# Simple-Robotics/LoIK

Measured on AMD Instinct MI355X. Metric: IK solves/sec to 1e-6 residual, Talos humanoid, batch=65536 per GPU, higher is better.
Workload: dtype f64

## Files before the change

loik_amd/csrc/loik_flat.hpp:

```cpp
#pragma once

#include "loik_lean.hpp"

namespace loikb {

constexpr int FLAT_RED = 8;
constexpr int FLAT_PART = 8;
constexpr int FLAT_JMP = 5;
constexpr int FLAT_MAXA = 16;
constexpr int FOLDW = 10;
constexpr int FLAT_COUNTERS_SLOT_HITS = 12;
constexpr int FLAT_NA_SMALL = 10;
constexpr int FSLOT_ROWS = 8;

struct FlatLane {
  int depth;
  int size;
  int jmp[FLAT_JMP];
  int anc[FLAT_MAXA];
  int red[FLAT_RED];
  int helper;
  int part[FLAT_PART];
};

enum : int { FC_LANE = 0, FC_B = 1, FC_Y = 7, FC_ATY = 13, FC_ATYW = 19, FC_ATBW = 25, FC_DY = 31, FC_DLT = 37, FC_ATYF = 43, FC_AW = 49, FC_A = 85,
              FC_VC = FC_DLT , FCD = 121 };
enum : int { FI_BNORM = 0, FI_TGIN, FI_STY, FI_TOLP, FI_TOLD, FI_DYQP, FI_ATDY, FI_UBP, FI_LBM, FI_C1, FI_C2, FI_PRIMAL, FI_DUAL, FI_DX,
             FI_DZ, FI_MULAST, FI_RED , FISC = FI_RED + 16 };

template <int NA>
__host__ __device__ constexpr int flat_xregion()
{
  int n = XROWS * 9;
  if (NA * WAVE + 2 > n) n = NA * WAVE + 2;
  if (WAVE * FOLDW > n) n = WAVE * FOLDW;
  return (n + 1) & ~1;
}
template <int NA> __host__ __device__ constexpr int flat_off_wl() { return flat_xregion<NA>(); }
template <int NA> __host__ __device__ constexpr int flat_off_nbuf() { return flat_off_wl<NA>() + 2 * (NA + 1) * WAVE; }
template <int NA> __host__ __device__ constexpr int flat_off_pbuf() { return flat_off_nbuf<NA>() + WAVE + 2; }
template <int NA> __host__ __device__ constexpr int flat_off_rbuf() { return flat_off_pbuf<NA>() + WAVE + 2; }
template <int NA> __host__ __device__ constexpr int flat_off_tail() { return flat_off_rbuf<NA>() + WAVE; }

template <typename T, int NA>
__host__ __device__ __forceinline__ size_t flat_lds_bytes(int nc, int G, bool a_shared, bool has_hv)
{
  (void)a_shared;
  const size_t per_inst = (size_t)nc * FCD + FISC;
  const size_t n = (size_t)flat_off_tail<NA>() + (has_hv ? (size_t)WAVE * 6 : 0) + (size_t)(WAVE / G) * per_inst;
  return (n * sizeof(T) + 15) & ~(size_t)15;
}

__device__ __forceinline__ size_t fslotA_at(int idx, int ndec, int dsl, int fblk, int G, int k, int jlane)
{
  (void)G;
  return ((size_t)idx * ndec + dsl) * fblk + (size_t)jlane * 8 + k;
}
__device__ __forceinline__ size_t fslotW_at(int idx, int ndec, int dsl, int fblk, int col)
{
  return ((size_t)idx * ndec + dsl) * fblk + col;
}

template <typename T>
__device__ __forceinline__ void se3_compose_left(const T* Ra, const T* ta, T* R, T* t)
{
  T Rn[9], tn[3];
#pragma unroll
  for (int i = 0; i < 3; ++i) {
#pragma unroll
    for (int j = 0; j < 3; ++j) Rn[3 * i + j] = Ra[3 * i] * R[j] + Ra[3 * i + 1] * R[3 + j] + Ra[3 * i + 2] * R[6 + j];
    tn[i] = ta[i] + Ra[3 * i] * t[0] + Ra[3 * i + 1] * t[1] + Ra[3 * i + 2] * t[2];
  }
#pragma unroll
  for (int k = 0; k < 9; ++k) R[k] = Rn[k];
#pragma unroll
  for (int k = 0; k < 3; ++k) t[k] = tn[k];
}

template <typename T>
__device__ __forceinline__ void flat_world_placement(T* xb, int lane, int jlane, const unsigned int* jrow4, int njmp, T* R, T* t)
{
#pragma unroll 1
  for (int r = 0; r < njmp; ++r) {
    {
      const int jr = (int)(((r < 4 ? jrow4[0] : jrow4[1]) >> (8 * (r & 3))) & 0xFFu);
      T Ra[9], ta[3];
      tail_sync();
      if (jlane < 9) xb[WAVE * 9 + jlane] = (jlane == 0 || jlane == 4 || jlane == 8) ? T(1) : T(0);
#pragma unroll
      for (int k = 0; k < 9; ++k) xb[lane * 9 + k] = R[k];
      tail_sync();
#pragma unroll
      for (int k = 0; k < 9; ++k) Ra[k] = xb[jr * 9 + k];
      tail_sync();
      if (jlane < 3) xb[WAVE * 9 + jlane] = T(0);
#pragma unroll
      for (int k = 0; k < 3; ++k) xb[lane * 9 + k] = t[k];
      tail_sync();
#pragma unroll
      for (int k = 0; k < 3; ++k) ta[k] = xb[jr * 9 + k];
      se3_compose_left(Ra, ta, R, t);
    }
  }
  tail_sync();
}

template <typename T>
__device__ __forceinline__ void flat_subtree_sum(T* rows, int lane, int jlane, int lim, int size, int nscan, const T* x, T* S)
{
  tail_sync();
  if (jlane < 6) rows[WAVE * 6 + jlane] = T(0);
  T B[6];
#pragma unroll
  for (int k = 0; k < 6; ++k) { B[k] = x[k]; S[k] = T(0); }
  int pos = lane;
  for (int k = 0; k < nscan; ++k) {
    tail_sync();
#pragma unroll
    for (int c = 0; c < 6; ++c) rows[lane * 6 + c] = B[c];
    tail_sync();
    const bool take = (size >> k) & 1;
    const int ra = take ? pos : WAVE;
    const int nx = lane + (1 << k);
    const int rb = nx < lim ? nx : WAVE;
    T a[6], b[6];
#pragma unroll
    for (int c = 0; c < 6; ++c) a[c] = rows[ra * 6 + c];
#pragma unroll
    for (int c = 0; c < 6; ++c) b[c] = rows[rb * 6 + c];
#pragma unroll
    for (int c = 0; c < 6; ++c) { S[c] += a[c]; B[c] += b[c]; }
    pos += take ? (1 << k) : 0;
  }
}

template <typename T>
__device__ __forceinline__ void flat_path_sum(T* rows, int lane, int jlane, const unsigned int* jrow4, int njmp, T* y)
{
  tail_sync();
  if (jlane < 6) rows[WAVE * 6 + jlane] = T(0);
#pragma unroll 1
  for (int r = 0; r < njmp; ++r) {
    {
      const int jr = (int)(((r < 4 ? jrow4[0] : jrow4[1]) >> (8 * (r & 3))) & 0xFFu);
      tail_sync();
#pragma unroll
      for (int c = 0; c < 6; ++c) rows[lane * 6 + c] = y[c];
      tail_sync();
      T a[6];
#pragma unroll
      for (int c = 0; c < 6; ++c) a[c] = rows[jr * 6 + c];
#pragma unroll
      for (int c = 0; c < 6; ++c) y[c] += a[c];
    }
  }
}

template <typename T>
__device__ __forceinline__ void actinv_force(const T* R, const T* t, const T* F, T* o)
{
  T c[3], d[3];
  cross3(t, F, c);
#pragma unroll
  for (int k = 0; k < 3; ++k) d[k] = F[3 + k] - c[k];
  mat3t_vec(R, F, o);
  mat3t_vec(R, d, o + 3);
}

template <typename T, int NMAX>
__device__ __forceinline__ void flat_fold8(T* rows, int lane, int gbase, int jlane, int lgG, const T* in, T* out)
{
  tail_sync();
  T* row = rows + lane * FOLDW;
#pragma unroll
  for (int q = 0; q < 8; ++q) row[q] = in[q];
  tail_sync();
  const int q = jlane & 7;
  const bool ismax = q < NMAX;
  const int nparts = 1 << (lgG - 3);
  {
    const T* col = rows + (gbase + (jlane >> 3)) * FOLDW + q;
    T a[8];
#pragma unroll
    for (int u = 0; u < 8; ++u) a[u] = col[u * nparts * FOLDW];
    const T m = tmax(tmax(tmax(a[0], a[1]), tmax(a[2], a[3])), tmax(tmax(a[4], a[5]), tmax(a[6], a[7])));
    T sm = a[0];
#pragma unroll
    for (int u = 1; u < 8; ++u) sm += a[u];
    row[8] = (NMAX >= 8 || ismax) ? m : sm;
  }
  tail_sync();
  {
    const T* col = rows + (gbase + q) * FOLDW + 8;
    T a[8];
#pragma unroll
    for (int p = 0; p < 8; ++p) a[p] = (p < 4 || lgG > 5) ? col[p * 8 * FOLDW] : T(0);
    const T m = tmax(tmax(tmax(a[0], a[1]), tmax(a[2], a[3])), tmax(tmax(a[4], a[5]), tmax(a[6], a[7])));
    T sm = a[0];
#pragma unroll
    for (int p = 1; p < 8; ++p) sm += a[p];
    row[9] = (NMAX >= 8 || ismax) ? m : sm;
  }
  tail_sync();
#pragma unroll
  for (int u = 0; u < 8; ++u) out[u] = rows[(gbase + u) * FOLDW + 9];
}

__device__ __forceinline__ unsigned int opaque(unsigned int x) { asm volatile("" : "+v"(x)); return x; }
// ... 538 lines not shown
      for (; kk + 2 < nscan; ++kk) {
        put_rows();
        tail_sync();
        scan_step(kk);
      }
      if (kk >= nscan) {
        tail_sync();
        part_v();
      } else {
        put_rows();
        tail_sync();
        const int wv = 1 << kk;
        const bool take0 = (size >> kk) & 1, take1 = (size >> (kk + 1)) & 1;
        const int p1 = pos + (take0 ? wv : 0);
        const int r0 = take0 ? pos : WAVE, r1 = take1 ? p1 : WAVE, r2 = take1 ? p1 + wv : WAVE;
        T a[6], b[6], c2[6];
#pragma unroll
        for (int c = 0; c < 6; ++c) a[c] = xb[r0 * 6 + c];
#pragma unroll
        for (int c = 0; c < 6; ++c) b[c] = xb[r1 * 6 + c];
#pragma unroll
        for (int c = 0; c < 6; ++c) c2[c] = xb[r2 * 6 + c];
        part_v();
#pragma unroll
        for (int c = 0; c < 6; ++c) SEn[c] += a[c] + (b[c] + c2[c]);
      }
      tail_sync();
      TAIL_TP(4)
#pragma unroll
      for (int k = 0; k < 6; ++k) Fw[k] = (P.rho + href_s) * SEn[k] - P.rho * SE[k];
      if (has_hv) {
#pragma unroll
        for (int k = 0; k < 6; ++k) Fw[k] -= shv[lane * 6 + k];
      }
      for (int c = 0; c < L.nc; ++c) {
        const T* c_ = cdi + c * cs;
        const T m = cmask(c);
#pragma unroll
        for (int k = 0; k < 6; ++k) Fw[k] += m * c_[FC_ATYF + k];
      }
      actinv_force(R0, t0, Fw, fi);
      si = dot6_halves(Sw, Fw);
#pragma unroll
      for (int k = 0; k < 6; ++k) SE[k] = SEn[k];
    }
    TAIL_TP(5)
    {
      T df[6];
#pragma unroll
      for (int k = 0; k < 6; ++k) df[k] = fi[k] - f[k];
      l_dfis = mass * inf6(df);
      si += w;
      l_stf = tabs(si);
      l_dstf = tabs(si - s);
      s = si;
#pragma unroll
      for (int k = 0; k < 6; ++k) f[k] = fi[k];
    }
    TAIL_TP(3)
    T red[8];
    {
      T in[8] = {tmax(l_prt, l_prs), tmax(l_dualv, l_stf), tmax(l_dvis, l_dnu), l_dz,
                 tmax(l_dfis, tmax(l_dyis, l_dw)), tmax(l_dg, l_dstf), l_up, l_lm};
      flat_fold8<T, 6>(xb, lane, gbase, jlane, lgG, in, red);
    }
    T ntol_p = T(0), ntol_d = T(0);
    if (P.tol_rel != T(0)) {
      T in2[8] = {tmax(l_av, l_nu), tmax(tmax(l_hrefv, l_g), l_stf), T(0), T(0), T(0), T(0), T(0), T(0)}, r2[8];
      flat_fold8<T, 8>(xb, lane, gbase, jlane, lgG, in2, r2);
      ntol_p = r2[0]; ntol_d = r2[1];
    }
    TAIL_TP(6)
    const T primal = red[0], dual = red[1], dx = red[2], dz = red[3], dyqp = red[4], atdy = red[5], ubp = red[6], lbm = red[7];
    const T mu_used = mu;
    const bool fixed = P.mode & MODE_FIXED_ITERS;
    const bool in_tail = (status & ST_TAIL) != 0;
    const bool logic = act && !fixed && !in_tail;
    const T tol_p = P.tol_abs + P.tol_rel * tmax(ntol_p, isc[FI_BNORM]);
    const T tol_d = P.tol_abs + P.tol_rel * tmax(ntol_d, P.Hv_inf_norm);
    const int itn = iter + (act ? 1 : 0);
    const bool conv = logic && (primal < tol_p) && (dual < tol_d);
    const bool feas_chk = logic && itn > 1;
    const bool c1 = atdy <= P.tol_primal_inf * dyqp, c2 = (ubp + lbm) <= P.tol_primal_inf * dyqp;
    const bool infeas = feas_chk && c1 && c2;
    const bool enter_tail = infeas && !conv;
    const bool upd = logic && !conv && !infeas;
    const bool mu_up = upd && (primal > T(10) * dual), mu_dn = upd && !mu_up && (dual > T(10) * primal);
    const bool tail_stop = !(dx >= P.tol_tail_solve || dz >= P.tol_tail_solve) || itn >= P.max_iter;
    const bool stop = act && (conv || ((enter_tail || in_tail) && tail_stop) || ((upd || fixed) && itn + 1 >= P.max_iter));
    iter = itn;
    status |= (conv ? ST_CONVERGED : 0) | (infeas ? ST_PRIMAL_INF : 0) | (enter_tail ? ST_TAIL : 0) | (stop ? ST_DONE : 0);
    tail_it = enter_tail ? 0 : (act && in_tail ? tail_it + 1 : tail_it);
    mu = mu_up ? mu * T(10) : (mu_dn ? mu * T(0.1) : mu);
    kexp += (mu_up ? 1 : 0) - (mu_dn ? 1 : 0);
    nflip += (mu_up || mu_dn) ? 1 : 0;
    done = done || stop;
    const bool finishing = stop;
    const bool leaving = done && has_inst;
    if (LOG) {
      T inl[8] = {l_prt, l_prs, l_stf, l_dualv, T(0), T(0), T(0), T(0)}, rl[8];
      flat_fold8<T, 8>(xb, lane, gbase, jlane, lgG, inl, rl);
      const int row = itn - 1;
      if (act && !in_tail && jlane == 0 && row < Bf.log_cap) {
        const double vals[9] = {(double)rl[0], (double)rl[1], (double)primal, (double)rl[2], (double)rl[3], (double)dual,
                                (double)mu_used, (double)(P.mu_scale * mu_used), (double)mu_used};
#pragma unroll
        for (int l = 0; l < 9; ++l) Bf.log[((size_t)l * Bf.log_B + lidx) * Bf.log_cap + row] = vals[l];
      }
    }
    if (__any(finishing || enter_tail)) {
      if ((finishing || enter_tail) && jlane == 0) {
        isc[FI_PRIMAL] = primal; isc[FI_DUAL] = dual; isc[FI_DX] = dx; isc[FI_DZ] = dz; isc[FI_MULAST] = mu_used;
        if (logic) { isc[FI_TOLP] = tol_p; isc[FI_TOLD] = tol_d; }
        if (feas_chk) {
          isc[FI_C1] = (T)(c1 ? 1 : 0); isc[FI_C2] = (T)(c2 ? 1 : 0); isc[FI_DYQP] = dyqp; isc[FI_ATDY] = atdy; isc[FI_UBP] = ubp; isc[FI_LBM] = lbm;
        }
      }
    }
    if (__any(finishing)) {
      T in1[8] = {l_prt, l_prs, l_stf, l_dvis, l_dnu, l_dfis, l_dyis, l_dw}, in2[8] = {l_av, l_nu, l_hrefv, l_g, l_dualv, T(0), T(0), T(0)};
      T r1[8], r2[8];
      flat_fold8<T, 8>(xb, lane, gbase, jlane, lgG, in1, r1);
      flat_fold8<T, 8>(xb, lane, gbase, jlane, lgG, in2, r2);
      if (finishing && jlane == 0) {
#pragma unroll
        for (int k = 0; k < 8; ++k) isc[FI_RED + k] = r1[k];
#pragma unroll
        for (int k = 0; k < 5; ++k) isc[FI_RED + 8 + k] = r2[k];
      }
      tail_sync();
    }
    if (leaving) {
      store_instance();
      need_load = true;
    }
    TAIL_TP(7)
  }
#ifdef LOIKB_TAIL_PROF
  if (blockIdx.x == 0 && threadIdx.x == 0) {
    for (int k = 0; k < 8; ++k) g_tail_prof[k] = prof_[k];
    for (int k = 8; k < 12; ++k) g_tail_prof[2 + k] = prof_[k];
    g_tail_prof[8] = n_wave_iters;
    g_tail_prof[9] = (clock64() - clk0_) * 100000ull / (wall_clock64() - wall0_ + 1);
  }
#endif
  if (lane == 0) atomicAdd(&Bf.counters[5], n_wave_iters);
  if (jlane == 0) {
    atomicAdd(&Bf.counters[6], n_slot_loads >> 16);
    atomicAdd(&Bf.counters[FLAT_COUNTERS_SLOT_HITS], n_slot_hits);
    atomicOr(&Bf.counters[LEAN_DECADES_SEEN], n_slot_loads & 0xFFFFu);
  }
}

template <typename T, int NA>
__global__ void __launch_bounds__(WAVE)
k_fslots(const Params<T> P, const Bufs<T> Bf, const JointDesc* __restrict__ jd, const TailTopo* __restrict__ topo,
         const int* __restrict__ child_list, const FlatLane* __restrict__ fl, int maxdepth, int nanc, int frows, int njmp,
         const int* __restrict__ slots, int nslots, int G, T* __restrict__ fslots, int kexp_lo, int ndec, int dw0, int nw,
         unsigned int* __restrict__ fmask)
{
  extern __shared__ __attribute__((aligned(16))) unsigned char smem_raw[];
  const Layout& L = P.L;
  constexpr int HX = 22;
  T* xch = reinterpret_cast<T*>(smem_raw);
  T* swt = xch + (WAVE + 1) * HX;
  T* ata_l = swt + (WAVE + 1) * 6;
  T* mutab = ata_l + (size_t)(WAVE / G) * P.L.nc * 21;
  T* lb = xch;
  const int lane = threadIdx.x;
  const int ipw = WAVE / G;
  const int sub = lane / G, jlane = lane % G, gbase = sub * G;
  const int nblk = gridDim.x, xcd = blockIdx.x & 7, rnd = blockIdx.x >> 3;
  const int blk = xcd * (nblk >> 3) + (xcd < (nblk & 7) ? xcd : (nblk & 7)) + rnd;
  const int idx = blk * ipw + sub;
  const bool has_inst = idx < nslots;
  const bool isj_lane = jlane < L.nb;
  const bool isj = has_inst && isj_lane;
  const int jl = isj_lane ? jlane : 0;
  const int sidx = slots[has_inst ? idx : 0];
  char* ip = lane_ptr<T>(Bf.tiles, L, sidx);
  int depth, fcol, arow[NA];
  T Sw[6];
  bool has_parent;
  int cslot;
  T base0[21];
  {
    const JointDesc d = jd[jl + 1];
    const FlatLane F = fl[jlane];
    depth = isj_lane ? F.depth : 0;
    fcol = F.helper >> 8;
    has_parent = !(d.flags & JF_PARENT_ROOT);
    cslot = isj_lane ? d.cslot : -1;
    unsigned int jrow4[(FLAT_JMP + 3) / 4] = {0u, 0u};
#pragma unroll
    for (int r = 0; r < FLAT_JMP; ++r) jrow4[r >> 2] |= (unsigned int)(F.jmp[r] >= 0 ? gbase + F.jmp[r] : WAVE) << (8 * (r & 3));
#pragma unroll
    for (int k = 0; k < NA; ++k) arow[k] = (k < FLAT_MAXA && F.anc[k] >= 0) ? gbase + F.anc[k] : WAVE;
    const char* rec = ip + (size_t)jl * JREC * pair_bytes<T>();
    const typename Vec2<T>::type cs = ldp<T>(rec, JP_CS);
    T R0[9], t0[3];
    joint_xform<T>(d, rec, cs.x, cs.y, R0, t0);
    if (!isj_lane) {
#pragma unroll
      for (int k = 0; k < 9; ++k) R0[k] = (k % 4 == 0) ? T(1) : T(0);
#pragma unroll
      for (int k = 0; k < 3; ++k) t0[k] = T(0);
    }
    flat_world_placement<T>(xch, lane, jlane, jrow4, njmp, R0, t0);
    const bool rev = d.flags & JF_REVOLUTE;
    const int jflags_h = d.flags;
    const T pitch_h = (d.flags & JF_HELICAL) ? (T)d.pitch : T(0);
    T ax[3], ra3[3], c[3];
#pragma unroll
    for (int k = 0; k < 3; ++k) ax[k] = isj_lane ? (T)d.axis[k] : T(0);
    mat3_vec(R0, ax, ra3);
    cross3(t0, ra3, c);
#pragma unroll
    for (int k = 0; k < 3; ++k) { Sw[k] = rev ? c[k] : ra3[k]; Sw[3 + k] = rev ? ra3[k] : T(0); }
    if (jflags_h & JF_HELICAL) {
#pragma unroll
      for (int k = 0; k < 3; ++k) Sw[k] += pitch_h * ra3[k];
    }
#pragma unroll
    for (int k = 0; k < 6; ++k) swt[lane * 6 + k] = Sw[k];
    if (lane < 6) swt[WAVE * 6 + lane] = T(0);
    {
      const T mass = (!isj_lane || (d.flags & JF_MASSLESS)) ? T(0) : T(1);
      T hb[21];
#pragma unroll
      for (int a = 0; a < 6; ++a)
#pragma unroll
        for (int b2 = a; b2 < 6; ++b2)
          hb[sym(a, b2)] = mass * ((a == b2 ? P.rho : T(0)) + (P.href_tab ? P.href_tab[(size_t)(jl + 1) * HREF_ROW + 6 * a + b2] : P.Href[6 * a + b2]));
      congr_sym(R0, t0, hb, base0);
    }
    if (cslot >= 0) {
      const char* crec = ip + (size_t)(L.off_c + cslot * L.crec) * pair_bytes<T>();
      T at[21], atw[21];
      for (int k = 0; k < 21; ++k)
        at[k] = (P.mode & MODE_A_SHARED) ? Bf.uni[L.nc * 36 + cslot * 21 + k]
                                         : *reinterpret_cast<const T*>(crec + (size_t)(CP_ATA + k / 2) * pair_bytes<T>() + (k & 1) * sizeof(T));
      congr_sym(R0, t0, at, atw);
#pragma unroll
      for (int k = 0; k < 21; ++k) ata_l[(sub * L.nc + cslot) * 21 + k] = atw[k];
    }
  }
  const TailTopo tp = topo[jl + 1];
  constexpr int NCH_REG = 3;
  int chl[NCH_REG];
#pragma unroll
  for (int c = 0; c < NCH_REG; ++c) chl[c] = (isj_lane && c < tp.nchild) ? gbase + child_list[tp.child_start + c] : WAVE;
  if (lane < ndec && lane < 16) mutab[lane] = (T)flat_decade_mu((double)P.mu0, kexp_lo + lane);
  tail_sync();
  if (lane < HX) xch[WAVE * HX + lane] = T(0);
  if (fmask != nullptr && has_inst && jlane == 0) fmask[sidx] = (nw >= 32 ? 0xFFFFu : ((1u << nw) - 1u)) << dw0;
  {
    const int lag = maxdepth - depth;
    tail_sync();
    for (int st = 0; st < maxdepth + nw - 1; ++st) {
      const int dsl = dw0 + st - lag;
      const bool on = isj && depth > 0 && dsl >= dw0 && dsl < dw0 + nw;
      T hh[21];
#pragma unroll
      for (int k = 0; k < 21; ++k) hh[k] = base0[k];
      const bool any2 = __any(on && tp.nchild > 1), any3 = __any(on && tp.nchild > 2);
      if (on) {
#pragma unroll
        for (int c = 0; c < NCH_REG; ++c) {
          if ((c == 1 && !any2) || (c == 2 && !any3)) continue;
          const T* x = xch + chl[c] * HX;
#pragma unroll
          for (int k = 0; k < 21; ++k) hh[k] += x[k];
        }
#pragma unroll 1
        for (int c = NCH_REG; c < tp.nchild; ++c) {
          const T* x = xch + (gbase + child_list[tp.child_start + c]) * HX;
#pragma unroll
          for (int k = 0; k < 21; ++k) hh[k] += x[k];
        }
      }
      tail_sync();
      if (on) {
        const T mu = mutab[dsl];
        const T mu_eq = P.mu_scale * mu, mu_in = mu;
        if (cslot >= 0) {
          const T* at = ata_l + (sub * L.nc + cslot) * 21;
#pragma unroll
          for (int k = 0; k < 21; ++k) hh[k] += mu_eq * at[k];
        }
        T U[6], UD[6];
        symv(hh, Sw, U);
        const T dinv = T(1) / (dot6_halves(Sw, U) + mu_in);
#pragma unroll
        for (int k = 0; k < 6; ++k) UD[k] = U[k] * dinv;
#pragma unroll
        for (int k = 0; k < 6; ++k) fslots[fslotA_at(sidx, ndec, dsl, frows, G, k, jlane)] = UD[k];
        fslots[fslotA_at(sidx, ndec, dsl, frows, G, 6, jlane)] = dinv;
        if (has_parent) {
          T* x = xch + lane * HX;
#pragma unroll
          for (int a = 0; a < 6; ++a)
#pragma unroll
            for (int b2 = a; b2 < 6; ++b2) x[sym(a, b2)] = hh[sym(a, b2)] - UD[a] * U[b2];
        }
      }
      tail_sync();
    }
  }
  lb[NA * WAVE + lane] = T(0);
  __builtin_amdgcn_s_waitcnt(0);
  tail_sync();
  for (int dsl = dw0; dsl < dw0 + nw; ++dsl) {
    T UDw[6], dinv = T(0);
#pragma unroll
    for (int k = 0; k < 6; ++k) UDw[k] = isj ? fslots[fslotA_at(sidx, ndec, dsl, frows, G, k, jlane)] : T(0);
    if (isj) dinv = fslots[fslotA_at(sidx, ndec, dsl, frows, G, 6, jlane)];
    T Lc[NA], Wc[NA];
#pragma unroll
    for (int k = 0; k < NA; ++k) {
      Lc[k] = dot6_halves(swt + arow[k] * 6, UDw);
      Wc[k] = T(0);
    }
    tail_sync();
#pragma unroll
    for (int k = 0; k < NA; ++k) lb[k * WAVE + lane] = Lc[k];
    tail_sync();
#pragma unroll
    for (int k = NA - 1; k >= 0; --k) {
      T acc = Lc[k];
#pragma unroll
      for (int k2 = k + 1; k2 < NA; ++k2) acc += lb[k * WAVE + arow[k2]] * Wc[k2];
      Wc[k] = (k < depth - 1) ? -acc : T(0);
    }
    tail_sync();
    if (isj) {
      const size_t base = fslotW_at(sidx, ndec, dsl, frows, fcol);
#pragma unroll
      for (int k = 0; k < NA; ++k)
        if (k < depth - 1) fslots[base + k] = Wc[k];
      fslots[base + depth - 1] = dinv;
    }
  }
}

template <typename T>
__global__ void k_rebuild_ud(char* tiles, Layout L, const JointDesc* __restrict__ jd, const T* __restrict__ uni, T rho, T mu_scale,
                             const T* __restrict__ href_tab, int a_shared, int B, T* __restrict__ scratch)
{
  const int b = blockIdx.x * blockDim.x + threadIdx.x;
  if (b >= B) return;
  char* lp = lane_ptr<T>(tiles, L, b);
  char* srec = lp + (size_t)L.off_s * pair_bytes<T>();
  if (*elem_ptr<T>(srec, SP_TAG, 0) != T(-2)) return;
  const T mu = *elem_ptr<T>(srec, SP_ST, 1);
  const T mu_eq = mu_scale * mu, mu_in = mu;
  T* o = scratch + (size_t)b * L.nb * 21;
  for (int i = 1; i <= L.nb; ++i) {
    for (int r = 0; r < 6; ++r)
      for (int c = r; c < 6; ++c)
        o[(i - 1) * 21 + sym(r, c)] = (jd[i].flags & JF_MASSLESS) ? T(0) : ((r == c ? rho : T(0)) + href_tab[(size_t)i * HREF_ROW + 6 * r + c]);
    if (jd[i].cslot >= 0) {
      const int cs = jd[i].cslot;
      for (int k = 0; k < 21; ++k) {
        const T a = a_shared ? uni[L.nc * 36 + cs * 21 + k]
                             : *elem_ptr<T>(lp + (size_t)(L.off_c + cs * L.crec) * pair_bytes<T>(), CP_ATA + k / 2, k & 1);
        o[(i - 1) * 21 + k] += mu_eq * a;
      }
    }
  }
  for (int i = L.nb; i >= 1; --i) {
    const JointDesc d = jd[i];
    T hh[21], U[6], UD[6], R[9], t[3], part[21];
    for (int k = 0; k < 21; ++k) hh[k] = o[(i - 1) * 21 + k];
    const int a0 = (d.flags & JF_REVOLUTE) ? 3 : 0;
    const T ax0 = (T)d.axis[0], ax1 = (T)d.axis[1], ax2 = (T)d.axis[2];
    for (int k = 0; k < 6; ++k) U[k] = hh[sym(k, a0)] * ax0 + hh[sym(k, a0 + 1)] * ax1 + hh[sym(k, a0 + 2)] * ax2;
    T sus = ax0 * U[a0] + ax1 * U[a0 + 1] + ax2 * U[a0 + 2];
    if (d.flags & JF_HELICAL) {
      const T ph = (T)d.pitch;
      for (int k = 0; k < 6; ++k) U[k] += ph * (hh[sym(k, 0)] * ax0 + hh[sym(k, 1)] * ax1 + hh[sym(k, 2)] * ax2);
      sus = (ax0 * U[3] + ax1 * U[4] + ax2 * U[5]) + ph * (ax0 * U[0] + ax1 * U[1] + ax2 * U[2]);
    }
    const T dd = T(1) / (sus + mu_in);
    for (int k = 0; k < 6; ++k) UD[k] = U[k] * dd;
    char* rec = lp + (size_t)(i - 1) * JREC * pair_bytes<T>();
    st6<T>(rec, JP_UD, UD);
    st_hi<T>(rec, JP_R, dd);
    {
      T vv[6], ff[6], hv[6];
      ld6<T>(rec, JP_V, vv);
      ld6<T>(rec, JP_F, ff);
      symv(hh, vv, hv);
      for (int k = 0; k < 6; ++k) ff[k] -= hv[k];
      st6<T>(rec, JP_P, ff);
    }
    if (d.parent == 0) continue;
    for (int r = 0; r < 6; ++r)
      for (int c = r; c < 6; ++c) hh[sym(r, c)] -= UD[r] * U[c];
    const typename Vec2<T>::type cs = ldp<T>(rec, JP_CS);
    joint_xform<T>(d, rec, cs.x, cs.y, R, t);
    congr_sym(R, t, hh, part);
    for (int k = 0; k < 21; ++k) o[(d.parent - 1) * 21 + k] += part[k];
  }
  *elem_ptr<T>(srec, SP_TAG, 0) = mu;
  *elem_ptr<T>(srec, SP_ST, 0) = (T)((int)*elem_ptr<T>(srec, SP_ST, 0) | ST_PFULL);
}

}
```

loik_amd/csrc/loik_host.hip:

```cpp
#include "loik_device.hpp"
#include "loik_tail.hpp"
#include "loik_lean.hpp"
#include "loik_flat.hpp"
#include "loik_flat2.hpp"
#include "loik_passes.hpp"
#include "loik_pose.hpp"
#ifdef LOIKB_FLAT_SEPARATE_TU
#include "loik_flat_inst.hpp"
LOIKB_FLAT2_INSTANCES(LOIKB_FLAT2_DECL)
LOIKB_FLAT1_INSTANCES(LOIKB_FLAT1_DECL)
#ifdef LOIKB_TAIL_PROF
int loikb_flat_prof_read(unsigned long long* out, int which, int reset);
#endif
#endif

#include "../../include/loik_amd.h"
#include "../../include/loik_amd_pose.h"

#include <algorithm>
#include <chrono>
#include <cmath>
#include <cstdio>
#include <cstdlib>
#include <cstring>
// ... 1533 lines not shown
  else if (S->f32) pl.why_not_flat = "fp32 solver";
  else if (S->opt.flags & LOIKB_OPT_NO_H_CACHE) pl.why_not_flat = "LOIKB_OPT_NO_H_CACHE (no precomputed factors)";
  else if (flat_any_mu(S) && !flat_any_mu_ok(S))
    pl.why_not_flat = "OSQP penalty rule: mu is off the decade grid, and the in-wave builder is k_flat2's / k_flat1's (17..64 joints, fp64, no logging)";
  else if (S->nb <= 16) pl.why_not_flat = "a small robot (<= 16 joints): k_solve + k_tail are faster on its short solves";
  else if (S->nc > (flat_takes_diagonal(S) ? 10 : S->flat.G / 6)) pl.why_not_flat = "more task constraints than the flat engine's lanes update in one pass";
  else if (pl.flat_waves_cu < (flat_takes_diagonal(S) ? 4 : 6)) pl.why_not_flat = "constraint blocks leave too few wavefronts per CU in LDS";
  else pl.flat = true;
  const bool flat_usable = pl.flat && (!S->href_known || flat_takes_diagonal(S) || href_is_scalar(S));
  pl.tail_max = S->opt.tail_max_instances > 0 ? S->opt.tail_max_instances : ((pl.lean || flat_usable) ? (1 << 20) : 32768);
  const int ntiles = (S->B + WAVE - 1) / WAVE;
  pl.nchunks = (ntiles >= 512 && !pl.lean && !flat_usable) ? 2 : 1;
  if (S->tune.chunks > 0) pl.nchunks = S->tune.chunks;
  pl.nchunks = std::max(1, std::min(pl.nchunks, ntiles));
  {
    auto need_of = [&](const loikb_solver_impl::TeamSched& sc) {
      const int edge = std::max(std::max(sc.nslots, 1) * EDGE_ENT, sc.nw > 1 ? sc.nw * Norms<double>::NALL : 0);
      return (size_t)(edge + std::max(sc.nvslots, 1) * 6) * WAVE * S->esz;
    };
    pl.solve_lds_need = need_of(S->sched[0]);
    pl.solve_ok = pl.solve_lds_need <= (size_t)160 * 1024;
    if (!pl.solve_ok) { pl.tail_max = 1 << 20; pl.nchunks = 1; }
  }
  S->plan = pl;
}

static bool bushy_goes_on_chip(const loikb_solver_impl* S)
{
  return S->nb <= WAVE && S->opt.tail_max_instances >= 0 && S->opt.max_launch_iters <= 0 &&
         !(S->opt.flags & (LOIKB_OPT_NO_COMPACTION | LOIKB_OPT_NO_H_CACHE)) && S->B <= S->plan.tail_max && S->tune.direct_tail;
}

template <typename T>
int run_tail(loikb_solver_impl* S, Chunk* C, Params<T>& P, int cur, int n_cur, int n_live, double* ms_out,
             unsigned long long* iters_out, bool whole_set = false)
{
  loikb_solver_impl::Set& A = C->set[cur];
  const int nw = (n_cur + WAVE - 1) / WAVE;
  int G0 = 8;
  while (G0 < S->nb) G0 <<= 1;
  const bool small_flat = whole_set && cur == 0 && S->chunks.size() == 1 && sizeof(T) == 8 && S->tune.flat_split && flat_applicable(S) && (P.mode & MODE_CACHE_H) &&
                          ((G0 == F2G && S->flat.ok && S->flat.nanc <= FLAT_NA_SMALL) || G0 == WAVE) && n_cur <= S->tune.flat_small_batch &&
                          n_cur >= std::max(1, S->tune.flat_min_batch);
  if (whole_set && small_flat) {
  } else if (whole_set) {
    hipLaunchKernelGGL(k_list_iota, grid1(n_cur), dim3(256), 0, C->stream, C->d_slots, n_cur);
  } else {
    C->h_wave.resize(2 * (size_t)nw + 2);
    int* cnt = C->h_wave.data();
    int* off = cnt + nw + 1;
    HIPCHK(hipMemcpyAsync(cnt, A.wave_live, sizeof(int) * nw, hipMemcpyDeviceToHost, C->stream));
    HIPCHK(hipStreamSynchronize(C->stream));
    int total = 0;
    for (int w = 0; w < nw; ++w) { off[w] = total; total += cnt[w]; }
    if (total != n_live) { g_last_error = "tail: live count mismatch"; return LOIKB_ERR_STATE; }
    HIPCHK(hipMemcpyAsync(A.wave_off, off, sizeof(int) * nw, hipMemcpyHostToDevice, C->stream));
    hipLaunchKernelGGL(k_list_live<T>, dim3(nw), dim3(WAVE), 0, C->stream, A.tiles, S->L, n_cur, A.wave_off, C->d_slots);
  }
  HIPCHK(hipGetLastError());
  Bufs<T> Bf = make_bufs<T>(S, C, cur);
  P.B = n_cur;
  int G = 8;
  while (G < S->nb) G <<= 1;
  const int ipw = WAVE / G;
  int tw = S->tune.tail_waves;
  while (tw > 1 && tw * tail_lds_bytes<T>(S->nc, G) > 160 * 1024) --tw;
  const size_t lds = tw * tail_lds_bytes<T>(S->nc, G);
  if (lds > 160 * 1024) { g_last_error = "tail kernel: constraint data exceeds the LDS of a CU"; return LOIKB_ERR_ARG; }
  if (lds > 64 * 1024) {
    HIPCHK(hipFuncSetAttribute((const void*)k_tail<T, true>, hipFuncAttributeMaxDynamicSharedMemorySize, (int)lds));
    HIPCHK(hipFuncSetAttribute((const void*)k_tail<T, false>, hipFuncAttributeMaxDynamicSharedMemorySize, (int)lds));
  }
  const int cu_share = std::max(1, (int)(S->ncu * (TAIL_WAVES / tw) * ((double)C->B / (double)S->B) + 0.5));
  int n = n_live;
  double total_ms = 0.0;
  unsigned long long iters = 0;
  const bool trace = S->tune.trace;
  const int* list = C->d_slots;
  {
    int ndec = S->plan.ndec, kexp_lo = S->plan.kexp_lo;
    if (S->tune.lean_adapt && S->seen_hi >= S->seen_lo && !(S->opt.flags & LOIKB_OPT_FIXED_ITERS) && !S->opt.logging) {
      const int lo = std::max(kexp_lo, S->seen_lo - 1), hi = std::min(kexp_lo + ndec - 1, S->seen_hi + 1);
      if (hi >= lo) { kexp_lo = lo; ndec = hi - lo + 1; }
    }
    const int ndec_hist = ndec, kexp_lo_hist = kexp_lo;
    const size_t wave_lds = lean_lds_bytes<T>(S->nc, G, S->a_shared);
    const bool flat_one_per_wave = S->tune.flat_split && sizeof(T) == 8 && ((G == F2G && S->flat.ok && S->flat.nanc <= FLAT_NA_SMALL) || G == WAVE);
    const bool flat_ok = flat_applicable(S) && (P.mode & MODE_CACHE_H) && n >= (flat_one_per_wave ? std::max(1, S->tune.flat_min_batch) : 64);
    if (flat_ok) {
      const int nanc = S->flat.nanc;
      const bool small_na = nanc <= FLAT_NA_SMALL;
      const int frows = S->flat.fblk;
      const bool can_build2 = S->tune.flat_build && G == F2G && small_na && sizeof(T) == 8 && S->tune.flat_split && C->d_fmask != nullptr &&
                              !S->opt.logging && !S->per_link && href_is_scalar(S);
      int mur = flat_any_mu(S) ? 1 : (can_build2 ? 2 : 0);
      if (mur == 1) { ndec = 1; kexp_lo = 0; }
      if (mur == 2) { ndec = S->plan.ndec; kexp_lo = S->plan.kexp_lo; }
      const size_t need = (size_t)n_cur * ndec * frows * sizeof(T);
      if (need > C->fslots_bytes) { g_last_error = "internal: decade-slot buffer of the flat engine smaller than the chunk"; return LOIKB_ERR_STATE; }
      const int has_hv = S->Hv_inf_norm != 0.0;
      const size_t flds = small_na ? flat_lds_bytes<T, FLAT_NA_SMALL>(S->nc, G, S->a_shared, has_hv) : flat_lds_bytes<T, FLAT_MAXA>(S->nc, G, S->a_shared, has_hv);
      int lgG = 3;
      while ((1 << lgG) < G) ++lgG;
      const double cu_sh = std::max(1.0, S->ncu * ((double)C->B / (double)S->B));
      const int cap_lat = (int)std::min<size_t>(4, (160 * 1024) / flds) * (int)(cu_sh + 0.5);
      const bool split = S->tune.flat_split && G == F2G && small_na && sizeof(T) == 8;
      const bool one = S->tune.flat_split && G == WAVE && sizeof(T) == 8;
      P.max_launch_iters = S->opt.max_iter + 1;
      const int mode_keep = P.mode;
      if (whole_set && S->zero_state && S->tune.flat_zero_state) P.mode |= MODE_ZERO_STATE;
      const bool queue_ready = small_flat && C->queue_ready && n_cur == S->B;
      C->queue_ready = false;
      if (queue_ready) {}
      else if (small_flat) hipLaunchKernelGGL(k_queue_init_iota, grid1(std::max(C->ring_cap, NCOUNTERS)), dim3(256), 0, C->stream, C->d_ring, C->ring_cap, C->d_slots, n_cur, C->d_counters, NCOUNTERS);
      else HIPCHK(hipMemsetAsync(C->d_counters, 0, NCOUNTERS * sizeof(unsigned int), C->stream));
      const hipEvent_t ev_first = queue_ready ? S->ev_t0 : C->ev_k0;
      if (!queue_ready) HIPCHK(hipEventRecord(C->ev_k0, C->stream));
      const bool ordered = !small_flat && whole_set && list == C->d_slots && n == n_cur && (split || one) && order_usable(S, C, n_cur);
      const bool order_was_stale = ordered && C->order_epoch != S->inputs_epoch;
      if (C->order_holdoff > 0) --C->order_holdoff;
      if (ordered) HIPCHK(hipMemcpyAsync(C->d_slots, C->d_order, sizeof(int) * (size_t)n, hipMemcpyDeviceToDevice, C->stream));
      C->stats.flat_ordered += ordered ? 1 : 0;
      int dw0 = 0, nw = ndec;
      if (mur == 2) {
        int wlo = 0, whi = -1;
        int q = (split && !S->opt.logging) ? flat_slice_for(S, n, ordered) : 0;
        if (q > 0 && (C->d_park == nullptr || (size_t)n_cur * flat2_park_stride(S->nc, true) * sizeof(double) > C->park_bytes)) q = 0;
        const bool win_ok = q > 0 && C->d_park != nullptr;
        if (S->tune.flat_win_n > 0) { wlo = S->tune.flat_win_lo; whi = wlo + S->tune.flat_win_n - 1; }
        else if (S->tune.flat_build == 2 && win_ok && S->end_hist_n > 0) {
          unsigned long long cum = 0;
          int k03 = 99, k97 = 99;
          for (int k = 0; k < 32; ++k) {
            cum += S->end_hist[k];
            if (k03 == 99 && cum * 100 >= 3ull * S->end_hist_n) k03 = k - 16;
            if (k97 == 99 && cum * 100 >= 97ull * S->end_hist_n) k97 = k - 16;
          }
          wlo = std::min(0, k03); whi = std::max(0, k97);
        }
        else if (S->tune.flat_build == 2 && win_ok && n >= 49152) {
          wlo = 0; whi = 4;
        }
        const int lo = std::max(wlo, kexp_lo), hi = std::min(whi, kexp_lo + ndec - 1);
        if (hi >= lo && (hi - lo + 1) < ndec) { dw0 = lo - kexp_lo; nw = hi - lo + 1; }
        else if (S->tune.flat_build == 2) mur = 0;
      }
      if (mur == 0) {
        ndec = ndec_hist; kexp_lo = kexp_lo_hist;
        nw = ndec; dw0 = 0;
      }
      const int win_bits = (int)(((nw >= 16 ? 0xFFFFu : ((1u << nw) - 1u)) << dw0) & 0xFFFFu);
      if (ndec > 0) {
        const dim3 hgrid((unsigned)((n + ipw - 1) / ipw));
        const size_t slds = (std::max((size_t)(WAVE + 1) * 22, (size_t)((small_na ? FLAT_NA_SMALL : FLAT_MAXA) + 1) * WAVE) + (size_t)(WAVE + 1) * 6 +
                             (size_t)ipw * S->nc * 21 + 16) * sizeof(T);
        if (small_na)
          hipLaunchKernelGGL((k_fslots<T, FLAT_NA_SMALL>), hgrid, dim3(WAVE), slds, C->stream, P, Bf, (const JointDesc*)S->d_jd,
                             (const TailTopo*)S->d_topo, (const int*)S->d_child_list, (const FlatLane*)S->flat.d_lanes, S->maxdepth,
                             nanc, frows, S->flat.njmp, list, n, G, (T*)C->d_fslots, kexp_lo, ndec, dw0, nw,
                             mur == 2 ? C->d_fmask : (unsigned int*)nullptr);
        else
          hipLaunchKernelGGL((k_fslots<T, FLAT_MAXA>), hgrid, dim3(WAVE), slds, C->stream, P, Bf, (const JointDesc*)S->d_jd,
                             (const TailTopo*)S->d_topo, (const int*)S->d_child_list, (const FlatLane*)S->flat.d_lanes, S->maxdepth,
                             nanc, frows, S->flat.njmp, list, n, G, (T*)C->d_fslots, kexp_lo, ndec, dw0, nw,
                             mur == 2 ? C->d_fmask : (unsigned int*)nullptr);
        HIPCHK(hipGetLastError());
      }
      if (!small_flat) HIPCHK(hipEventRecord(C->ev_k2, C->stream));
      const int n_first = n;
      bool small_finish = false;
      dim3 grid((unsigned)std::min((n + ipw - 1) / ipw, cap_lat));
      {
        if (!small_flat) hipLaunchKernelGGL(k_ring_fill, grid1(C->ring_cap), dim3(256), 0, C->stream, C->d_ring, C->ring_cap, list, n, C->d_counters);
        if (split || one) {
          if (C->d_aux == nullptr) HIPCHK(hipMalloc((void**)&C->d_aux, 4 * sizeof(void*)));
          const void* auxh[4] = {S->d_topo, S->d_child_list, C->d_fmask, nullptr};
          if (memcmp(auxh, C->aux_h, sizeof(auxh)) != 0) {
            memcpy(C->aux_h, auxh, sizeof(auxh));
            HIPCHK(hipStreamSynchronize(C->stream));
            HIPCHK(hipMemcpy(C->d_aux, C->aux_h, sizeof(auxh), hipMemcpyHostToDevice));
          }
        }
        if (split) {
          const size_t lds2 = flat2_lds_bytes<FLAT_NA_SMALL>(S->nc, has_hv != 0, mur == 1);
          int per_cu = (int)std::min<size_t>((size_t)8, (160 * 1024) / lds2);
          if (S->tune.lean_wg_per_cu > 0) per_cu = std::min(per_cu, S->tune.lean_wg_per_cu);
          grid = dim3((unsigned)std::min(n, per_cu * (int)(cu_sh + 0.5)));
          const int resident = (int)grid.x;
          const size_t park_need = (size_t)n_cur * flat2_park_stride(S->nc, true) * sizeof(double);
          (void)resident;
          int quantum = flat_slice_for(S, n, ordered);
          if (quantum > 0 && (C->d_park == nullptr || park_need > C->park_bytes)) quantum = 0;
#define LOIKB_LAUNCH_FLAT2(...)                                                                                                 \
  hipLaunchKernelGGL((k_flat2<FLAT_NA_SMALL, ##__VA_ARGS__>), grid, dim3(WAVE), lds2, C->stream,                                 \
                     *reinterpret_cast<const Params<double>*>(&P), *reinterpret_cast<const Bufs<double>*>(&Bf),                  \
                     (const JointDesc*)S->d_jd, (const FlatLane*)S->flat.d_lanes, nanc, S->flat.nscan, S->flat.njmp, C->d_ring, n, \
                     (const double*)C->d_fslots, frows, kexp_lo, ndec, (double)S->Href[0], (int)((unsigned int)has_hv | ((unsigned int)(S->maxdepth & 0xFF) << 8) | ((unsigned int)win_bits << 16)), C->ring_cap - 1, quantum,       \
                     (double*)C->d_park, flat2_park_stride(S->nc, true), (const void* const*)C->d_aux)
          const int hm = S->per_link ? 3 : href_is_scalar(S) ? 0 : href_is_diagonal(S) ? 1 : 2;
          if (mur == 1) {
            if (S->tune.flat_slice < 0) quantum = 0;
            if (hm == 3) { quantum = 0; LOIKB_LAUNCH_FLAT2(false, 3, false, 1); }
            else if (hm == 2) { quantum = 0; LOIKB_LAUNCH_FLAT2(false, 2, false, 1); }
            else if (hm == 1) { quantum = 0; LOIKB_LAUNCH_FLAT2(false, 1, false, 1); }
            else if (quantum > 0) LOIKB_LAUNCH_FLAT2(true, 0, false, 1);
            else LOIKB_LAUNCH_FLAT2(false, 0, false, 1);
          }
          else if (mur == 2) {
            if (quantum > 0) LOIKB_LAUNCH_FLAT2(true, 0, false, 2); else LOIKB_LAUNCH_FLAT2(false, 0, false, 2);
          }
          else if (S->opt.logging) {
            quantum = 0;
            if (hm == 3) LOIKB_LAUNCH_FLAT2(false, 3, true);
            else if (hm >= 1) LOIKB_LAUNCH_FLAT2(false, 2, true);
            else LOIKB_LAUNCH_FLAT2(false, 0, true);
          }
          else if (hm == 3) { if (quantum > 0) LOIKB_LAUNCH_FLAT2(true, 3); else LOIKB_LAUNCH_FLAT2(false, 3); }
          else if (hm == 2) { if (quantum > 0) LOIKB_LAUNCH_FLAT2(true, 2); else LOIKB_LAUNCH_FLAT2(false, 2); }
          else if (hm == 1) { if (quantum > 0) LOIKB_LAUNCH_FLAT2(true, 1); else LOIKB_LAUNCH_FLAT2(false, 1); }
          else if (quantum > 0) LOIKB_LAUNCH_FLAT2(true);
          else LOIKB_LAUNCH_FLAT2();
#undef LOIKB_LAUNCH_FLAT2
        } else if (one) {
          auto lds_of = [&](int bufs) { return small_na ? flat1_lds_bytes<FLAT_NA_SMALL>(S->nc, has_hv != 0, bufs) : flat1_lds_bytes<FLAT_MAXA>(S->nc, has_hv != 0, bufs); };
          const int one_buf = mur != 1 && std::min<size_t>(8, (160 * 1024) / lds_of(1)) > std::min<size_t>(8, (160 * 1024) / lds_of(2));
          const size_t lds1 = lds_of(one_buf ? 1 : 2);
          int per_cu1 = (int)std::min<size_t>(8, (160 * 1024) / lds1);
          if (S->tune.lean_wg_per_cu > 0) per_cu1 = std::min(per_cu1, S->tune.lean_wg_per_cu);
          grid = dim3((unsigned)std::min(n, per_cu1 * (int)(cu_sh + 0.5)));
          const int resident = (int)grid.x, full = per_cu1 * (int)(cu_sh + 0.5);
          (void)resident; (void)full;
          const int quantum = mur == 1 ? 0 : flat_slice_for(S, n, ordered);
#define LOIKB_LAUNCH_FLAT1(NAV, ...)                                                                                            \
  hipLaunchKernelGGL((k_flat1<NAV, ##__VA_ARGS__>), grid, dim3(WAVE), lds1, C->stream,                                          \
                     *reinterpret_cast<const Params<double>*>(&P), *reinterpret_cast<const Bufs<double>*>(&Bf),                  \
                     (const JointDesc*)S->d_jd, (const FlatLane*)S->flat.d_lanes, nanc, S->flat.nscan, S->flat.njmp, C->d_ring, n, \
                     (const double*)C->d_fslots, frows, kexp_lo, ndec, (double)S->Href[0], has_hv | (one_buf ? 2 : 0) | ((S->maxdepth & 0xFF) << 8),  \
                     C->ring_cap - 1, quantum, (const void* const*)C->d_aux)
          const int hm = S->per_link ? 3 : href_is_scalar(S) ? 0 : href_is_diagonal(S) ? 1 : 2;
          if (mur == 1) {
            if (hm == 3) { if (small_na) LOIKB_LAUNCH_FLAT1(FLAT_NA_SMALL, false, 3, false, 1); else LOIKB_LAUNCH_FLAT1(FLAT_MAXA, false, 3, false, 1); }
            else if (hm >= 1) { if (small_na) LOIKB_LAUNCH_FLAT1(FLAT_NA_SMALL, false, 2, false, 1); else LOIKB_LAUNCH_FLAT1(FLAT_MAXA, false, 2, false, 1); }
            else if (small_na) LOIKB_LAUNCH_FLAT1(FLAT_NA_SMALL, false, 0, false, 1);
            else LOIKB_LAUNCH_FLAT1(FLAT_MAXA, false, 0, false, 1);
          }
          else if (S->opt.logging) {
            const int quantum = 0;
            if (hm == 3) { if (small_na) LOIKB_LAUNCH_FLAT1(FLAT_NA_SMALL, false, 3, true); else LOIKB_LAUNCH_FLAT1(FLAT_MAXA, false, 3, true); }
            else if (hm >= 1) { if (small_na) LOIKB_LAUNCH_FLAT1(FLAT_NA_SMALL, false, 2, true); else LOIKB_LAUNCH_FLAT1(FLAT_MAXA, false, 2, true); }
            else if (small_na) LOIKB_LAUNCH_FLAT1(FLAT_NA_SMALL, false, 0, true);
            else LOIKB_LAUNCH_FLAT1(FLAT_MAXA, false, 0, true);
          }
          else if (hm == 3) {
            if (quantum > 0) { if (small_na) LOIKB_LAUNCH_FLAT1(FLAT_NA_SMALL, true, 3); else LOIKB_LAUNCH_FLAT1(FLAT_MAXA, true, 3); }
            else if (small_na) LOIKB_LAUNCH_FLAT1(FLAT_NA_SMALL, false, 3);
            else LOIKB_LAUNCH_FLAT1(FLAT_MAXA, false, 3);
          } else if (hm == 2) {
            if (quantum > 0) { if (small_na) LOIKB_LAUNCH_FLAT1(FLAT_NA_SMALL, true, 2); else LOIKB_LAUNCH_FLAT1(FLAT_MAXA, true, 2); }
            else if (small_na) LOIKB_LAUNCH_FLAT1(FLAT_NA_SMALL, false, 2);
            else LOIKB_LAUNCH_FLAT1(FLAT_MAXA, false, 2);
          } else if (hm == 1) {
            if (quantum > 0) { if (small_na) LOIKB_LAUNCH_FLAT1(FLAT_NA_SMALL, true, 1); else LOIKB_LAUNCH_FLAT1(FLAT_MAXA, true, 1); }
            else if (small_na) LOIKB_LAUNCH_FLAT1(FLAT_NA_SMALL, false, 1);
            else LOIKB_LAUNCH_FLAT1(FLAT_MAXA, false, 1);
          } else if (quantum > 0) { if (small_na) LOIKB_LAUNCH_FLAT1(FLAT_NA_SMALL, true); else LOIKB_LAUNCH_FLAT1(FLAT_MAXA, true); }
          else if (small_na) LOIKB_LAUNCH_FLAT1(FLAT_NA_SMALL);
          else LOIKB_LAUNCH_FLAT1(FLAT_MAXA);
#undef LOIKB_LAUNCH_FLAT1
        } else {
#define LOIKB_LAUNCH_FLAT(NAV, ...)                                                                                             \
  hipLaunchKernelGGL((k_flat<T, NAV, ##__VA_ARGS__>), grid, dim3(WAVE), flds, C->stream, P, Bf, (const JointDesc*)S->d_jd,                \
                     (const FlatLane*)S->flat.d_lanes, nanc, S->flat.nscan, S->flat.njmp, (const int*)C->d_ring, n, lgG,          \
                     (const T*)C->d_fslots, frows, kexp_lo, ndec, (T)S->Href[0], has_hv)
        if (S->opt.logging) { if (small_na) LOIKB_LAUNCH_FLAT(FLAT_NA_SMALL, true); else LOIKB_LAUNCH_FLAT(FLAT_MAXA, true); }
        else if (small_na) LOIKB_LAUNCH_FLAT(FLAT_NA_SMALL);
        else LOIKB_LAUNCH_FLAT(FLAT_MAXA);
#undef LOIKB_LAUNCH_FLAT
        }
        HIPCHK(hipGetLastError());
        P.mode = mode_keep;
        int* nxt = (list == C->d_slots) ? C->d_slots2 : C->d_slots;
        small_finish = small_flat && S->tune.small_finish;
        if (small_finish)
          hipLaunchKernelGGL(k_small_finish<T>, dim3(1), dim3(256), 0, C->stream, A.tiles, S->L, list, n, nxt, C->d_counters, NCOUNTERS, C->h_counters);
        else
          hipLaunchKernelGGL(k_list_unfinished<T>, grid1(n), dim3(256), 0, C->stream, A.tiles, S->L, list, n, nxt, C->d_counters + 3);
        HIPCHK(hipGetLastError());
        C->stats.launches++;
        C->stats.tail_launches++;
        C->stats.lean_launches++;
        C->stats.flat_launches++;
        if (split) C->stats.flat_split_launches++;
      }
      int* next = (list == C->d_slots) ? C->d_slots2 : C->d_slots;
      HIPCHK(hipEventRecord(C->ev_k1, C->stream));
      const bool order_pass = !small_flat && S->tune.flat_order && whole_set && n_first == n_cur && (split || one) && !(S->opt.flags & LOIKB_OPT_FIXED_ITERS);
      if (!order_pass && !small_finish) HIPCHK(hipMemcpyAsync(C->h_counters, C->d_counters, NCOUNTERS * sizeof(unsigned int), hipMemcpyDeviceToHost, C->stream));
      if (order_pass) {
        HIPCHK(hipMemsetAsync(C->d_order_bins, 0, sizeof(unsigned int) * 2 * ORDER_BINS, C->stream));
        hipLaunchKernelGGL(k_order_count<T>, grid1(n_cur), dim3(256), 0, C->stream, A.tiles, S->L, n_cur, S->opt.max_iter, C->d_order_bins,
                           C->d_counters + ORDER_DEC_HIST);
        HIPCHK(hipMemcpyAsync(C->h_counters, C->d_counters, NCOUNTERS * sizeof(unsigned int), hipMemcpyDeviceToHost, C->stream));
        hipLaunchKernelGGL(k_order_scan, dim3(1), dim3(ORDER_BINS), 0, C->stream, C->d_order_bins);
        hipLaunchKernelGGL(k_order_scatter<T>, grid1(n_cur), dim3(256), 0, C->stream, A.tiles, S->L, n_cur, S->opt.max_iter, C->d_order_bins, C->d_order);
        HIPCHK(hipGetLastError());
        C->order_n = n_cur;
        C->order_epoch = S->inputs_epoch;
      }
      HIPCHK(hipStreamSynchronize(C->stream));
      float ms = 0.f, t0 = 0.f, hms = 0.f;
      HIPCHK(hipEventElapsedTime(&ms, ev_first, C->ev_k1));
      if (!queue_ready) HIPCHK(hipEventElapsedTime(&t0, S->ev_t0, C->ev_k0));
      if (!small_flat) HIPCHK(hipEventElapsedTime(&hms, ev_first, C->ev_k2));
      iters += C->h_counters[1];
      if (C->h_counters[FLAT_COUNTERS_ERR]) {
        g_last_error = (C->h_counters[FLAT_COUNTERS_ERR] & 4u) ? "internal: the flat engine's dynamic LDS does not start at LDS address 0 (lds_abs)"
                                                               : "internal: a wavefront of the flat engine gave up waiting on its work queue";
        return LOIKB_ERR_STATE;
// ... 1829 lines not shown
```

Measured before the change: 7.068 million.

## Keep per-decade UD/dinv factors in registers across chunked decade windows in k_fslots

The fslots kernel now processes the decade window in chunks of up to four decades. For large grids it keeps each lane's UD/dinv results in a register array instead of writing them to global memory and reading them back after a full s_waitcnt. It also reads the joint-axis vector from shared memory instead of holding it in registers, and sets an amdgpu_waves_per_eu occupancy hint. The cost is more passes of the depth pipeline (one per chunk), more register pressure from the udr array, and an extra CREG template instantiation selected on the host by grid size.

```diff
diff --git a/loik_amd/csrc/loik_flat.hpp b/loik_amd/csrc/loik_flat.hpp
--- a/loik_amd/csrc/loik_flat.hpp
+++ b/loik_amd/csrc/loik_flat.hpp
@@ -12,6 +12,7 @@
 constexpr int FLAT_COUNTERS_SLOT_HITS = 12;
 constexpr int FLAT_NA_SMALL = 10;
 constexpr int FSLOT_ROWS = 8;
+constexpr int FSLOT_NWR = 4;
 
 struct FlatLane {
   int depth;
@@ -51,9 +52,8 @@
   return (n * sizeof(T) + 15) & ~(size_t)15;
 }
 
-__device__ __forceinline__ size_t fslotA_at(int idx, int ndec, int dsl, int fblk, int G, int k, int jlane)
-{
-  (void)G;
+__device__ __forceinline__ size_t fslotA_at(int idx, int ndec, int dsl, int fblk, int k, int jlane)
+{
   return ((size_t)idx * ndec + dsl) * fblk + (size_t)jlane * 8 + k;
 }
 __device__ __forceinline__ size_t fslotW_at(int idx, int ndec, int dsl, int fblk, int col)
@@ -898,8 +898,8 @@
   }
 }
 
-template <typename T, int NA>
-__global__ void __launch_bounds__(WAVE)
+template <typename T, int NA, bool CREG>
+__global__ void __launch_bounds__(WAVE) __attribute__((amdgpu_waves_per_eu(NA <= FLAT_NA_SMALL ? 2 : 1)))
 k_fslots(const Params<T> P, const Bufs<T> Bf, const JointDesc* __restrict__ jd, const TailTopo* __restrict__ topo,
          const int* __restrict__ child_list, const FlatLane* __restrict__ fl, int maxdepth, int nanc, int frows, int njmp,
          const int* __restrict__ slots, int nslots, int G, T* __restrict__ fslots, int kexp_lo, int ndec, int dw0, int nw,
@@ -1000,12 +1000,15 @@
   tail_sync();
   if (lane < HX) xch[WAVE * HX + lane] = T(0);
   if (fmask != nullptr && has_inst && jlane == 0) fmask[sidx] = (nw >= 32 ? 0xFFFFu : ((1u << nw) - 1u)) << dw0;
-  {
-    const int lag = maxdepth - depth;
+  T udr[FSLOT_NWR][7];
+  const int lag = maxdepth - depth;
+  const int cw = CREG ? FSLOT_NWR : nw;
+  for (int c0 = dw0; c0 < dw0 + nw; c0 += cw) {
+    const int cn = (dw0 + nw - c0) < cw ? (dw0 + nw - c0) : cw;
     tail_sync();
-    for (int st = 0; st < maxdepth + nw - 1; ++st) {
-      const int dsl = dw0 + st - lag;
-      const bool on = isj && depth > 0 && dsl >= dw0 && dsl < dw0 + nw;
+    for (int st = 0; st < maxdepth + cn - 1; ++st) {
+      const int dsl = c0 + st - lag;
+      const bool on = isj && depth > 0 && dsl >= c0 && dsl < c0 + cn;
       T hh[21];
 #pragma unroll
       for (int k = 0; k < 21; ++k) hh[k] = base0[k];
@@ -1034,14 +1037,26 @@
 #pragma unroll
           for (int k = 0; k < 21; ++k) hh[k] += mu_eq * at[k];
         }
-        T U[6], UD[6];
-        symv(hh, Sw, U);
-        const T dinv = T(1) / (dot6_halves(Sw, U) + mu_in);
+        T U[6], UD[6], Sl[6];
+#pragma unroll
+        for (int k = 0; k < 6; ++k) Sl[k] = CREG ? swt[lane * 6 + k] : Sw[k];
+        symv(hh, Sl, U);
+        const T dinv = T(1) / (dot6_halves(Sl, U) + mu_in);
 #pragma unroll
         for (int k = 0; k < 6; ++k) UD[k] = U[k] * dinv;
-#pragma unroll
-        for (int k = 0; k < 6; ++k) fslots[fslotA_at(sidx, ndec, dsl, frows, G, k, jlane)] = UD[k];
-        fslots[fslotA_at(sidx, ndec, dsl, frows, G, 6, jlane)] = dinv;
+        if constexpr (CREG) {
+          const int w = dsl - c0;
+#pragma unroll
+          for (int w2 = 0; w2 < FSLOT_NWR; ++w2) {
+#pragma unroll
+            for (int k = 0; k < 6; ++k) udr[w2][k] = (w2 == w) ? UD[k] : udr[w2][k];
+            udr[w2][6] = (w2 == w) ? dinv : udr[w2][6];
+          }
+        } else {
+#pragma unroll
+          for (int k = 0; k < 6; ++k) fslots[fslotA_at(sidx, ndec, dsl, frows, k, jlane)] = UD[k];
+          fslots[fslotA_at(sidx, ndec, dsl, frows, 6, jlane)] = dinv;
+        }
         if (has_parent) {
           T* x = xch + lane * HX;
 #pragma unroll
@@ -1052,39 +1067,52 @@
       }
       tail_sync();
     }
-  }
-  lb[NA * WAVE + lane] = T(0);
-  __builtin_amdgcn_s_waitcnt(0);
-  tail_sync();
-  for (int dsl = dw0; dsl < dw0 + nw; ++dsl) {
-    T UDw[6], dinv = T(0);
-#pragma unroll
-    for (int k = 0; k < 6; ++k) UDw[k] = isj ? fslots[fslotA_at(sidx, ndec, dsl, frows, G, k, jlane)] : T(0);
-    if (isj) dinv = fslots[fslotA_at(sidx, ndec, dsl, frows, G, 6, jlane)];
-    T Lc[NA], Wc[NA];
-#pragma unroll
-    for (int k = 0; k < NA; ++k) {
-      Lc[k] = dot6_halves(swt + arow[k] * 6, UDw);
-      Wc[k] = T(0);
-    }
+    lb[NA * WAVE + lane] = T(0);
+    if constexpr (!CREG) __builtin_amdgcn_s_waitcnt(0);
     tail_sync();
-#pragma unroll
-    for (int k = 0; k < NA; ++k) lb[k * WAVE + lane] = Lc[k];
-    tail_sync();
-#pragma unroll
-    for (int k = NA - 1; k >= 0; --k) {
-      T acc = Lc[k];
-#pragma unroll
-      for (int k2 = k + 1; k2 < NA; ++k2) acc += lb[k * WAVE + arow[k2]] * Wc[k2];
-      Wc[k] = (k < depth - 1) ? -acc : T(0);
-    }
-    tail_sync();
-    if (isj) {
-      const size_t base = fslotW_at(sidx, ndec, dsl, frows, fcol);
-#pragma unroll
-      for (int k = 0; k < NA; ++k)
-        if (k < depth - 1) fslots[base + k] = Wc[k];
-      fslots[base + depth - 1] = dinv;
+#pragma unroll 1
+    for (int dsl = c0; dsl < c0 + cn; ++dsl) {
+      T UDw[6], dinv = T(0);
+#pragma unroll
+      for (int k = 0; k < 6; ++k) UDw[k] = T(0);
+      if constexpr (CREG) {
+        const int w = dsl - c0;
+#pragma unroll
+        for (int w2 = 0; w2 < FSLOT_NWR; ++w2) {
+#pragma unroll
+          for (int k = 0; k < 6; ++k) UDw[k] = (isj && w2 == w) ? udr[w2][k] : UDw[k];
+          dinv = (isj && w2 == w) ? udr[w2][6] : dinv;
+        }
+      } else {
+#pragma unroll
+        for (int k = 0; k < 6; ++k) UDw[k] = isj ? fslots[fslotA_at(sidx, ndec, dsl, frows, k, jlane)] : T(0);
+        if (isj) dinv = fslots[fslotA_at(sidx, ndec, dsl, frows, 6, jlane)];
+      }
+      T Lc[NA], Wc[NA];
+#pragma unroll
+      for (int k = 0; k < NA; ++k) {
+        Lc[k] = dot6_halves(swt + arow[k] * 6, UDw);
+        Wc[k] = T(0);
+      }
+      tail_sync();
+#pragma unroll
+      for (int k = 0; k < NA; ++k) lb[k * WAVE + lane] = Lc[k];
+      tail_sync();
+#pragma unroll
+      for (int k = NA - 1; k >= 0; --k) {
+        T acc = Lc[k];
+#pragma unroll
+        for (int k2 = k + 1; k2 < NA; ++k2) acc += lb[k * WAVE + arow[k2]] * Wc[k2];
+        Wc[k] = (k < depth - 1) ? -acc : T(0);
+      }
+      tail_sync();
+      if (isj) {
+        const size_t base = fslotW_at(sidx, ndec, dsl, frows, fcol);
+#pragma unroll
+        for (int k = 0; k < NA; ++k)
+          if (k < depth - 1) fslots[base + k] = Wc[k];
+        fslots[base + depth - 1] = dinv;
+      }
     }
   }
 }
diff --git a/loik_amd/csrc/loik_host.hip b/loik_amd/csrc/loik_host.hip
--- a/loik_amd/csrc/loik_host.hip
+++ b/loik_amd/csrc/loik_host.hip
@@ -1709,18 +1709,16 @@
       const int win_bits = (int)(((nw >= 16 ? 0xFFFFu : ((1u << nw) - 1u)) << dw0) & 0xFFFFu);
       if (ndec > 0) {
         const dim3 hgrid((unsigned)((n + ipw - 1) / ipw));
+        const bool creg = hgrid.x >= 2048;
         const size_t slds = (std::max((size_t)(WAVE + 1) * 22, (size_t)((small_na ? FLAT_NA_SMALL : FLAT_MAXA) + 1) * WAVE) + (size_t)(WAVE + 1) * 6 +
                              (size_t)ipw * S->nc * 21 + 16) * sizeof(T);
-        if (small_na)
-          hipLaunchKernelGGL((k_fslots<T, FLAT_NA_SMALL>), hgrid, dim3(WAVE), slds, C->stream, P, Bf, (const JointDesc*)S->d_jd,
-                             (const TailTopo*)S->d_topo, (const int*)S->d_child_list, (const FlatLane*)S->flat.d_lanes, S->maxdepth,
-                             nanc, frows, S->flat.njmp, list, n, G, (T*)C->d_fslots, kexp_lo, ndec, dw0, nw,
-                             mur == 2 ? C->d_fmask : (unsigned int*)nullptr);
-        else
-          hipLaunchKernelGGL((k_fslots<T, FLAT_MAXA>), hgrid, dim3(WAVE), slds, C->stream, P, Bf, (const JointDesc*)S->d_jd,
-                             (const TailTopo*)S->d_topo, (const int*)S->d_child_list, (const FlatLane*)S->flat.d_lanes, S->maxdepth,
-                             nanc, frows, S->flat.njmp, list, n, G, (T*)C->d_fslots, kexp_lo, ndec, dw0, nw,
-                             mur == 2 ? C->d_fmask : (unsigned int*)nullptr);
+#define LOIKB_LAUNCH_FSLOTS(NA, CREG)                                                                                              \
+  hipLaunchKernelGGL((k_fslots<T, NA, CREG>), hgrid, dim3(WAVE), slds, C->stream, P, Bf, (const JointDesc*)S->d_jd,                  \
+                     (const TailTopo*)S->d_topo, (const int*)S->d_child_list, (const FlatLane*)S->flat.d_lanes, S->maxdepth, nanc, frows,  \
+                     S->flat.njmp, list, n, G, (T*)C->d_fslots, kexp_lo, ndec, dw0, nw, mur == 2 ? C->d_fmask : (unsigned int*)nullptr)
+        if (small_na) { if (creg) LOIKB_LAUNCH_FSLOTS(FLAT_NA_SMALL, true); else LOIKB_LAUNCH_FSLOTS(FLAT_NA_SMALL, false); }
+        else { if (creg) LOIKB_LAUNCH_FSLOTS(FLAT_MAXA, true); else LOIKB_LAUNCH_FSLOTS(FLAT_MAXA, false); }
+#undef LOIKB_LAUNCH_FSLOTS
         HIPCHK(hipGetLastError());
       }
       if (!small_flat) HIPCHK(hipEventRecord(C->ev_k2, C->stream));
```

New measurement: 7.164 million (median of 6 runs). 1.01x the previous value.
